# ntu-caokun/DIRECT

Measured on AMD Instinct MI355X. Metric: ddp_iterations_per_sec, higher is better.
Workload: dtype f64

## Files before the change

direct_amd/abi.py:

```python
import ctypes as C

import numpy as np

NX = 9
NU = 10
P_LIMIT = 128

DIRECT_OK = 0
DIRECT_ERR_INVALID = 1
DIRECT_ERR_UNSUPPORTED = 2
DIRECT_ERR_DEVICE = 3
DIRECT_ERR_NO_DEVICE = 4

F32 = 0
F64 = 1
MEM_HOST = 0
MEM_DEVICE = 1

RTN_DONE = 0
RTN_FEAS_OPT = 1
RTN_FEAS_FOUND = 2
RTN_NEG_TIME = -3
RTN_BP_STUCK = -4
RTN_INVALID = -100
# ... 170 lines not shown
class ClusterCorridorOut(C.Structure):
    _fields_ = [("mem", C.c_int32), ("reserved", C.c_int32), ("n_seg", C.c_void_p), ("n_planes", C.c_void_p), ("planes", C.c_void_p),
                ("seeds", C.c_void_p), ("centers", C.c_void_p), ("rtn", C.c_void_p)]


CLUSTER_CORRIDOR_OUTPUTS = ("n_seg", "n_planes", "planes", "seeds", "centers", "rtn")
CLUSTER_CORRIDOR_ARGTYPES = (C.c_void_p, C.c_void_p, C.c_void_p, C.c_void_p)
CLUSTER_CORRIDOR_STATS = ("rounds", "due_seeds", "unique_seeds", "pops")


class LaunchInfo(C.Structure):
    _fields_ = [
        ("dynamic", C.c_int32), ("shared_search", C.c_int32), ("pair_trials", C.c_int32), ("single_steps", C.c_int32),
        ("n_buffers", C.c_int32), ("resident_waves", C.c_int32), ("batch", C.c_int32), ("shared_sweep", C.c_int32),
        ("bwd_knot_visits", C.c_uint64), ("fwd_knot_visits", C.c_uint64),
        ("half_tickets", C.c_int32), ("reserved", C.c_int32),
    ]


class Config(C.Structure):
    _fields_ = [
        ("dtype", C.c_int32), ("device", C.c_int32), ("max_batch", C.c_int32),
        ("n_seg_max", C.c_int32), ("p_max", C.c_int32), ("reserved", C.c_int32),
    ]


FLAG_STATIC_SCHEDULE, FLAG_YIELD = 1, 2


def phase0_params(**kw):
    d = dict(max_vel=2.0, max_acc=2.0, w_snap=1.0, w_terminal=1.0, w_time=1.0, iter_max=50,
# ... 119 lines not shown
```

direct_amd/csrc/ddp_wave.h:

```cpp
#pragma once
#include <stdint.h>

#include "ddp_tables.h"
#include "sched_ticket.h"

#if defined(DIRECT_EMULATE)
#include <cmath>
#include <cstdio>
#include <cstdlib>
#include <cstring>
namespace direct {
using std::fabs; using std::fma; using std::fmax; using std::fmin; using std::log; using std::pow; using std::sqrt;
inline int& emu_lane() { static thread_local int l = 64; return l; }
template <typename T>
inline T* uniform_ptr(T* p) { return p; }
template <typename T>
inline T emu_uniform(T x, int line) {
  static thread_local unsigned char seen[4096][sizeof(double)];
  const int l = emu_lane();
  if (l >= 64) return x;
  unsigned char* ref = seen[line & 4095];
  if (l == 0) {
    std::memcpy(ref, &x, sizeof(T));
  } else if (std::memcmp(ref, &x, sizeof(T)) != 0 && !(x != x)) {
// ... 1075 lines not shown
      if (lane < 9) L.z[lane] = ldx(Xp(buf, N), lane) - (Real)B.xd[(size_t)b * 9 + lane];
    }
    WSYNC();
    const double pterm = terminal_sq();
    WSYNC();
    LANES { LV(slog) = LV(plog).value(); }
    st.costq = qsum;
    st.cost = qsum + 0.5 * B.k.w_term * pterm;
    st.sumlog = WAVE_SUM_D(slog);
    st.errsum = WAVE_SUM_D(serr);
    st.viol = WAVE_SUM_I(nviol);
    st.npos = WAVE_SUM_I(npos);
    st.neg_time = neg;
  }

  DDP_DEV void reset_filter() {
    double logcost = st.cost - st.mu * st.sumlog;
    double err = 0.0;
    if (st.infeas) {
      err = st.errsum;
      if (err < B.k.tol) err = 0.0;
    }
    st.logcost = logcost;
    st.err = err;
    double* f = B.filt + (size_t)b * B.fcap * 2;
    f[0] = logcost;
    f[1] = err;
    st.nfilter = 1;
    st.step = 0;
    st.fp_failed = 0;
// ... 44 lines not shown
          Tk = (Real)2 * Tk;
          cnt++;
        } else {
          vio = 0;
        }
        WSYNC();
      }
      LANES {
        if (lane >= 9 && lane < 18) stx(Xp(0, l), lane, L.z[lane]);
        if (lane == 18) stx(Xp(0, l), 18, Tk);
      }
      WSYNC();
    }
  }

  DDP_DEV void begin() {
    N = B.n_seg[b];
    int bad_sizes = (N < 1 || N > B.nmax) ? 1 : 0;
    if (!bad_sizes) {
      PLV(int, badp);
      LANES {
        LV(badp) = 0;
        for (int k = lane; k < N; k += 64) {
          const int np = np_(k);
          if (np < 1 || np > B.pmax || np > Lds::kPMax) LV(badp) = 1;
        }
      }
      bad_sizes = WAVE_ANY(badp);
    }
    if (bad_sizes) {
      N = 0;
      LANES {
        int* dst = (int*)&L.st;
        for (int e = lane; e < (int)(sizeof(TrajState) / 4); e += 64) dst[e] = 0;
      }
      WSYNC();
      st.rtn = -100;
      st.done = 1;
      st.line_failed = 1;
      return;
    }
    st.nseg = N;
    st.cur = 0;
    st.infeas = B.infeas_in ? (int)B.infeas_in[b] : 0;
    st.infeas_ref = st.infeas;
    st.line_failed = 1;
    const St* T0 = B.T0 + (size_t)b * B.nmax;
    LANES {
      if (lane < 9) stx(Xp(0, 0), lane, (Real)B.x0[(size_t)b * 9 + lane]);
      for (int k = lane; k < N; k += 64) {
        St* rec = Xp(0, k);
        Real T = T0[k];
        if (B.k.zero_init || (B.init_bez == nullptr && B.init_poly == nullptr)) {
          for (int a = 0; a < 9; a++) stx(rec, 9 + a, (Real)0);
        } else if (B.init_poly != nullptr) {
          const St* row = B.init_poly + ((size_t)b * B.nmax + k) * 18;
          for (int a = 0; a < 9; a++) stx(rec, 9 + a, (Real)row[9 + a]);
        } else {
          const St* row = B.init_bez + ((size_t)b * B.nmax + k) * 18;
          for (int i = 3; i < 6; i++)
            for (int d = 0; d < 3; d++) {
              Real acc = 0;
              for (int l = 0; l < 6; l++) acc += (Real)kBez2Mono[l][i] * (T * (Real)row[d * 6 + l]);
              stx(rec, 9 + (i - 3) * 3 + d, acc / powi(T, i));
            }
        }
        stx(rec, 18, T);
      }
    }
    if (!B.k.zero_init && B.k.line_init) line_init();
    for (int k = 0; k < N; k++) {
      const int nc = 6 * np_(k) + 55;
      LANES {
        for (int i = 0; i < RPL; i++) {
          int r = lane + 64 * i;
          if (r < nc) {
            Sp_(B.S[0], k)[r] = (St)0.1;
            Sp_(B.Y[0], k)[r] = (St)0.01;
          }
        }
      }
    }
    WSYNC();
    eval_sweep(0, true);
    if (B.k.line_init && st.npos == 0 && st.infeas) {
      st.infeas = 0;
      eval_sweep(0, false);
    }
    st.prev_cost = st.cost;
    st.nc0 = 6 * np_(0) + 55;
    st.mu = st.cost / (double)N / (double)st.nc0;
    reset_filter();
    st.reg = B.k.line_init ? 10 : 0;
    st.bp_failed = 0;
    st.opterr = 0.0;
    st.stepsize = 0.0;
    st.rtn = 0;
    st.iter = 0;
    st.done = 0;
    st.bp_no_upd = 0;
    st.no_upd = 0;
    st.fwd_passes = 0;
// ... 2463 lines not shown
```

direct_amd/csrc/direct_ddp.hip:

```cpp
#include <hip/hip_runtime.h>

#include <cmath>
#include <cstdio>
#include <cstdlib>
#include <cstring>
#include <string>
#include <vector>

#include "../../include/direct_ddp.h"
#include "ddp_wave.h"
#include "traj_sample.h"
#include "traj_eval.h"
#include "traj_audit.h"
#include "corridor_io.h"
#include "host_stage.h"
#include "rccl_gather.h"

using namespace direct;

#if defined(DDP_TIMING)
#undef DDP_TICK_OBJ
#define DDP_TICK_OBJ W
#endif
#ifndef DDP_WAVES_F32
// ... 7 lines not shown
#define DDP_WAVES_WIDE 2
#endif
#ifndef DDP_WAVES_WIDER
#define DDP_WAVES_WIDER 1
#endif
template <typename St>
struct MinWaves { static constexpr int v = DDP_WAVES_F32; };
template <>
struct MinWaves<double> { static constexpr int v = DDP_WAVES_F64; };

template <typename St>
__device__ __forceinline__ int traj_of(const Batch<St>& B, int i) {
  return B.idx ? __builtin_amdgcn_readfirstlane(B.idx[i]) : i;
}

template <typename St, int RPL>
__global__ __launch_bounds__(64) void k_begin(Batch<St> B) {
  __shared__ WaveLds<Cmp, St, RPL> lds;
  Wave<Cmp, St, RPL> W(B, lds, traj_of(B, blockIdx.x));
  W.init_tables();
  W.begin();
  W.store_state();
}

template <typename St, int RPL>
__global__ __launch_bounds__(64, (RPL > 7 ? DDP_WAVES_WIDER : (RPL > 4 ? DDP_WAVES_WIDE : MinWaves<St>::v))) void k_iterate(Batch<St> B, int n_iters) {
  __shared__ WaveLds<Cmp, St, RPL> lds;
  Wave<Cmp, St, RPL> W(B, lds, traj_of(B, blockIdx.x));
  W.load_state();
  if (__builtin_amdgcn_readfirstlane(lds.st.done)) return;
  W.init_tables();
  W.iterate(n_iters);
  W.store_state();
}

constexpr int kDoneBit = 1 << 30;
#ifndef DDP_POLL_SLEEP
// ... 219 lines not shown
}

template <typename St, int RPL>
__global__ __launch_bounds__(64) void k_stuck(Batch<St> B) {
  __shared__ WaveLds<Cmp, St, RPL> lds;
  Wave<Cmp, St, RPL> W(B, lds, traj_of(B, blockIdx.x));
  W.load_state();
  if (__builtin_amdgcn_readfirstlane(lds.st.rtn) != kRtnStuckPending) return;
  W.init_tables();
  W.stuck_tail();
  W.store_state();
}

template <typename St, int RPL>
__global__ __launch_bounds__(64) void k_finish(Batch<St> B, OutPtrs<St> O, const int* sched_err) {
  __shared__ WaveLds<Cmp, St, RPL> lds;
  Wave<Cmp, St, RPL> W(B, lds, traj_of(B, blockIdx.x));
  W.load_state();
  W.init_tables();
  if (__builtin_amdgcn_readfirstlane(*sched_err)) lds.st.rtn = -101;
  finish_wave(W, O);
}

template <typename St, int RPL>
__global__ __launch_bounds__(64) void k_field(Batch<St> B, int field, St* buf, int set) {
  __shared__ WaveLds<Cmp, St, RPL> lds;
  Wave<Cmp, St, RPL> W(B, lds, traj_of(B, blockIdx.x));
  W.load_state();
  W.init_tables();
  if (set) {
// ... 163 lines not shown
  int* live = nullptr;
  unsigned long long* visits = nullptr;
  direct_ddp_launch_info_t last_info = {};
  int sched_slots = 0;
  int slots_cap = 0;
  int sched_chunk = 1;
  int sched_half = -1;
  int pair_trials = -1;
  int sched_prio = 1;
  int sched_tail = 8;
  int yield_k = 0;
  int* nwaves = nullptr;
  int* sched_dbg = nullptr;
  int* sched_mark = nullptr;
  bool dynamic = true;
  int B = 0;
  bool begun = false;
  direct_ddp_params_t params = {};
  direct_ddp_batch_in_t cur_in = {};
  std::vector<void*> allocs;
};

template <typename T>
static direct_status_t dalloc(direct_ddp_handle_t h, T** p, size_t bytes) {
  hipError_t e = hs::alloc_all(h->allocs, {hs::want(p, bytes)});
  if (e != hipSuccess) return fail(DIRECT_ERR_DEVICE, std::string("hipMalloc: ") + hipGetErrorString(e));
  return DIRECT_OK;
}
#define TRY(expr)                            \
  do {                                       \
// ... 88 lines not shown
  switch (rpl) {
#define OCC_CASE(R) case R: e = hipOccupancyMaxActiveBlocksPerMultiprocessor(&per_cu, k_iterate_dyn<Real, R>, 64, 0); break;
    OCC_CASE(2) OCC_CASE(3) OCC_CASE(4) OCC_CASE(5) OCC_CASE(6) OCC_CASE(7) OCC_CASE(8) OCC_CASE(10) OCC_CASE(12)
#undef OCC_CASE
    default: e = hipOccupancyMaxActiveBlocksPerMultiprocessor(&per_cu, k_iterate_dyn<Real, 14>, 64, 0);
  }
#endif
  int v = (e == hipSuccess && per_cu > 0) ? per_cu * h->n_cu : 0;
  if (h->slots_cap > 0 && v > h->slots_cap) v = h->slots_cap;
  h->slots_of[rpl] = v > 0 ? v : -1;
  return v;
}

template <typename Real>
static void launch_begin_t(direct_ddp_handle_t h) {
  for (const auto& c : batch_classes(h)) {
    auto Bt = make_batch<Real>(h, h->cur_in, h->params, c);
    RPL_LAUNCH(c.rpl, h->stream, k_begin, Real, c.cnt, Bt);
  }
}
static hipStream_t class_stream(direct_ddp_handle_t h, size_t ci, size_t n_classes) {
  if (n_classes <= 1 || ci >= 12) return h->stream;
  if (!h->fork_ev && hipEventCreateWithFlags(&h->fork_ev, hipEventDisableTiming) != hipSuccess) return h->stream;
  if (!h->cstream[ci]) {
    if (hipStreamCreateWithFlags(&h->cstream[ci], hipStreamNonBlocking) != hipSuccess ||
        hipEventCreateWithFlags(&h->cev[ci], hipEventDisableTiming) != hipSuccess) {
      h->cstream[ci] = nullptr;
      return h->stream;
    }
  }
  return h->cstream[ci];
}
template <typename Real>
static void launch_iterate_t(direct_ddp_handle_t h, int n, int mode) {
  const auto classes = batch_classes(h);
  (void)hipMemsetAsync(h->visits, 0, 4 * sizeof(unsigned long long), h->stream);
  direct_ddp_launch_info_t& li = h->last_info;
  li = direct_ddp_launch_info_t{};
  li.n_buffers = h->nbuf; li.batch = h->B;
  if (mode == 0) {
    (void)hipMemsetAsync(h->tickets, 0, 16 * sizeof(int), h->stream);
    (void)hipMemsetAsync(h->sched + 2, 0, (size_t)h->B * sizeof(int), h->stream);
    if (h->help) (void)hipMemsetAsync(h->help, 0, (size_t)h->B * sizeof(HelpSlot), h->stream);
    if (h->bshare && h->bshare_mode != 0) {
      const size_t nb = (size_t)(h->B < h->bshare_cap ? h->B : h->bshare_cap);
      (void)hipMemsetAsync(h->bshare, 0, nb * sizeof(BwdShare), h->stream);
      (void)hipMemsetAsync(h->bflag, 0, nb * h->nmax * sizeof(int), h->stream);
    }
  }
  bool forked = false;
  if (mode == 0 && classes.size() > 1 && class_stream(h, 0, classes.size()) != h->stream) {
    (void)hipEventRecord(h->fork_ev, h->stream);
    forked = true;
  }
  int biggest = -1;
  for (size_t ci = 0; ci < classes.size(); ci++) {
    const auto& c = classes[ci];
    auto Bt = make_batch<Real>(h, h->cur_in, h->params, c);
// ... 55 lines not shown
      S.half = h->sched_half > 0 ? 1 : 0;
      S.chunk = S.half ? 1 : h->sched_chunk;
      S.prio = h->sched_prio;
      S.tail = help ? h->sched_tail : 0;
      S.dbg = h->sched_dbg;
#if defined(DDP_SCHED_DEBUG)
      S.mark = nullptr; S.grid = slots;
      if (slots <= 8192) { S.mark = h->sched_mark; Bt.mark = h->sched_mark; (void)hipMemsetAsync(h->sched_mark, 0, 2 * 8192 * sizeof(int), st); }
#endif
      S.waves = h->nwaves + (ci < 16 ? ci : 15);
      S.alive = h->live + (ci < 16 ? ci : 15);
      S.yield_k = h->yield_k;
      S.yield_min = 64;
      if (h->yield_k > 0) {
        S.tail = 0;
        (void)hipMemsetD32Async((hipDeviceptr_t)S.waves, slots, 1, st);
        (void)hipMemsetD32Async((hipDeviceptr_t)S.alive, c.cnt, 1, st);
      }
      if (help) {
        Bt.help = h->help;
        Bt.help_early = h->help_early;
        int* live = h->live + (ci < 16 ? ci : 15);
        (void)hipMemsetD32Async((hipDeviceptr_t)live, c.cnt, 1, st);
        Bt.live = live;
        Bt.tail_thresh = h->single_ratio > 0 ? slots / h->single_ratio : 0;
        if (is_big) { li.shared_search = 1; li.single_steps = Bt.k.pair_trials ? 0 : 1; }
        if (sweep_ok && h->bshare_mode != 0 && h->bshare_mode != 2 && S.chunk == 1 && (h->bshare_mode > 0 || 8 * c.cnt <= slots)) {
          Bt.bshare = h->bshare; Bt.bflag = h->bflag; Bt.brec = h->brec; Bt.bforce = 0; Bt.bvisits = h->visits + 2;
          if (is_big) li.shared_sweep = 1;
        }
      }
      if (is_big) { li.dynamic = 1; li.half_tickets = S.half; }
      if (Bt.bshare) {
        publish(Bt);
        switch (c.rpl) {
          case 2: hipLaunchKernelGGL((k_iterate_dyn<Real, 2, true>), dim3(slots), dim3(64), 0, st, Bt, n, S); break;
#if !defined(DDP_DEV_RPL2)
          case 3: hipLaunchKernelGGL((k_iterate_dyn<Real, 3, true>), dim3(slots), dim3(64), 0, st, Bt, n, S); break;
          default: hipLaunchKernelGGL((k_iterate_dyn<Real, 4, true>), dim3(slots), dim3(64), 0, st, Bt, n, S);
#endif
        }
      } else {
        RPL_LAUNCH(c.rpl, st, k_iterate_dyn, Real, slots, Bt, n, S);
      }
    } else {
      Bt.bshare = nullptr;
      if (is_big && li.shared_sweep) li.shared_sweep = 0;
      RPL_LAUNCH(c.rpl, st, k_iterate, Real, c.cnt, Bt, n);
    }
    {
      auto Bs = make_batch<Real>(h, h->cur_in, h->params, c);
      Bs.visits = h->visits;
      RPL_LAUNCH(c.rpl, st, k_stuck, Real, c.cnt, Bs);
    }
    if (forked && st != h->stream) {
      (void)hipEventRecord(h->cev[ci], st);
      (void)hipStreamWaitEvent(h->stream, h->cev[ci], 0);
    }
  }
}
template <typename Real>
static void launch_field_t(direct_ddp_handle_t h, int field, int set) {
  for (const auto& c : batch_classes(h)) {
    auto Bt = make_batch<Real>(h, h->cur_in, h->params, c);
    RPL_LAUNCH(c.rpl, h->stream, k_field, Real, c.cnt, Bt, field, (Real*)h->fieldbuf, set);
// ... 5 lines not shown
  const bool dev = out->mem == DIRECT_MEM_DEVICE;
#define PICK(f) (dev ? out->f : (out->f ? h->o.f : nullptr))
  O.rtn = PICK(rtn); O.iter_used = PICK(iter_used); O.fwd_passes = PICK(fwd_passes);
  O.infeas_out = PICK(infeas_out); O.line_failed_out = PICK(line_failed_out);
  O.cost = (Real*)PICK(cost); O.costq = (Real*)PICK(costq); O.jerk_cost = (Real*)PICK(jerk_cost);
  O.terminal_norm2 = (Real*)PICK(terminal_norm2); O.opterr = (Real*)PICK(opterr); O.mu = (Real*)PICK(mu);
  O.bez = (Real*)PICK(bez); O.poly = (Real*)PICK(poly); O.T = (Real*)PICK(T);
#undef PICK
  return O;
}
template <typename Real>
static void launch_finish_t(direct_ddp_handle_t h, const direct_ddp_batch_out_t* out) {
  auto O = out_ptrs<Real>(h, out);
  for (const auto& c : batch_classes(h)) {
    auto Bt = make_batch<Real>(h, h->cur_in, h->params, c);
    RPL_LAUNCH(c.rpl, h->stream, k_finish, Real, c.cnt, Bt, O, (const int*)(h->sched + 1));
  }
}

static direct_status_t staged_upload(direct_ddp_handle_t h, hs::Stage& st, const char* name) {
  const hipError_t e = hs::stage_upload(st, h->stage, h->stream);
  return e == hipSuccess ? DIRECT_OK : fail(DIRECT_ERR_DEVICE, std::string(name) + ": staging: " + hipGetErrorString(e));
}
static direct_status_t staged_finish(direct_ddp_handle_t h, const hs::Stage& st, const char* name) {
  hipError_t e = hs::stage_download(st, h->stream, hipGetLastError());
  if (st.host) e = hs::drain(h->stream, e);
  return e == hipSuccess ? DIRECT_OK : fail(DIRECT_ERR_DEVICE, std::string(name) + ": " + hipGetErrorString(e));
}
static direct_status_t workspace(direct_ddp_handle_t h, hs::Block& ws, size_t bytes, const char* name) {
  const hipError_t e = hs::grow(ws, h->stream, bytes);
  return e == hipSuccess ? DIRECT_OK : fail(DIRECT_ERR_DEVICE, std::string("workspace of ") + name + ": " + hipGetErrorString(e));
// ... 225 lines not shown
  A(&h->best_idx, 16); A(&h->best_cost, 16);
  A(&h->sched, (B + 2) * sizeof(int));
  A(&h->visits, 4 * sizeof(unsigned long long));
  A(&h->live, 16 * sizeof(int));
  A(&h->nwaves, 16 * sizeof(int));
  A(&h->sched_mark, 2 * 8192 * sizeof(int));
  A(&h->sched_dbg, 64 * sizeof(int));
  if (st == DIRECT_OK && hipMemset(h->sched_dbg, 0, 64 * sizeof(int)) != hipSuccess) st = fail(DIRECT_ERR_DEVICE, "hipMemset");
  A(&h->tickets, 16 * sizeof(int));
  A(&h->order, B * sizeof(int32_t)); A(&h->cls_dev, B * sizeof(int32_t));
  if (const char* ev = getenv("DIRECT_DDP_CHUNK")) h->sched_chunk = atoi(ev) > 0 ? atoi(ev) : 1;
  if (const char* ev = getenv("DIRECT_DDP_HALF")) h->sched_half = atoi(ev) > 0 ? 1 : 0;
  if (const char* ev = getenv("DIRECT_DDP_PRIO")) h->sched_prio = atoi(ev);
  if (const char* ev = getenv("DIRECT_DDP_TAIL")) h->sched_tail = std::max(0, std::min(atoi(ev), 64));
  if (const char* ev = getenv("DIRECT_DDP_PAIR")) h->pair_trials = atoi(ev);
  h->fieldbuf_bytes = B * nm * (size_t)std::max(ncm, 100) * r + B * 16 * r + B * 9 * r;
  A(&h->fieldbuf, h->fieldbuf_bytes);
  if (st == DIRECT_OK && (hipEventCreate(&h->ev0) != hipSuccess || hipEventCreate(&h->ev1) != hipSuccess ||
                          hs::create(h->sample_ev) != hipSuccess || hs::create(h->eval_ev) != hipSuccess ||
                          hs::create(h->audit_ev) != hipSuccess))
    st = fail(DIRECT_ERR_DEVICE, "hipEventCreate failed");
  if (st == DIRECT_OK && hipMemset(h->sched, 0, (B + 2) * sizeof(int)) != hipSuccess)
    st = fail(DIRECT_ERR_DEVICE, "hipMemset failed");
  if (st != DIRECT_OK) {
    direct_ddp_destroy(h);
    return st;
  }
  *out = h;
  return DIRECT_OK;
}
// ... 132 lines not shown
    HIP_TRY(up(h->x0, in->x0, B * 9 * r)); d.x0 = h->x0;
    HIP_TRY(up(h->xd, in->xd, B * 9 * r)); d.xd = h->xd;
    if (in->T0) { HIP_TRY(up(h->T0, in->T0, B * nm * r)); d.T0 = h->T0; }
    HIP_TRY(up(h->n_planes, in->n_planes, B * nm * 4)); d.n_planes = h->n_planes;
    HIP_TRY(up(h->planes, in->planes, B * nm * h->pmax * 4 * r)); d.planes = h->planes;
    if (in->init_bez) { HIP_TRY(up(h->init_bez, in->init_bez, B * nm * 18 * r)); d.init_bez = h->init_bez; }
    if (in->init_poly) { HIP_TRY(up(h->init_poly, in->init_poly, B * nm * 18 * r)); d.init_poly = h->init_poly; }
    if (in->seeds) { HIP_TRY(up(h->seeds, in->seeds, B * nm * 3 * r)); d.seeds = h->seeds; }
    if (in->infeas_in) { HIP_TRY(up(h->infeas_in, in->infeas_in, B)); d.infeas_in = h->infeas_in; }
    if (packed) {
      HIP_TRY(hipMemcpyAsync(h->in_blob, h->in_host, h->in_blob_bytes, hipMemcpyHostToDevice, h->stream));
      HIP_TRY(hipEventRecord(h->in_ev, h->stream));
      h->in_ev_pending = true;
    }
  }
  if (!in->infeas_in) {
    HIP_TRY(hipMemsetAsync(h->infeas_in, p->infeas ? 1 : 0, B, h->stream));
    d.infeas_in = h->infeas_in;
  }
  if (!in->T0) {
    const int n = (int)(B * nm);
    if (h->dtype == DIRECT_F64)
      hipLaunchKernelGGL(k_time_alloc<double>, dim3((n + 255) / 256), dim3(256), 0, h->stream, (int)B, (int)nm, d.n_seg, (const double*)d.x0,
                         (const double*)d.xd, (const double*)d.seeds, p->max_vel, p->max_acc, (double*)h->T0);
    else
      hipLaunchKernelGGL(k_time_alloc<float>, dim3((n + 255) / 256), dim3(256), 0, h->stream, (int)B, (int)nm, d.n_seg, (const float*)d.x0,
                         (const float*)d.xd, (const float*)d.seeds, p->max_vel, p->max_acc, (float*)h->T0);
    HIP_TRY(hipGetLastError());
    d.T0 = h->T0;
  }
  if (fresh) {
    h->B = in->batch;
    TRY(classify_batch(h, in->mem == DIRECT_MEM_HOST ? in : &d, in->mem == DIRECT_MEM_HOST));
  }
  if (fresh) HIP_TRY(hipMemsetAsync(h->sched + 1, 0, sizeof(int), h->stream));
  d.mem = DIRECT_MEM_DEVICE;
  h->cur_in = d;
  h->params = *p;
  h->B = in->batch;
  if (p->iter_max + 4 > h->fcap) {
    if (h->filt) { HIP_TRY(hipStreamSynchronize(h->stream)); HIP_TRY(hipFree(h->filt)); h->filt = nullptr; }
    h->fcap = p->iter_max + 4;
    HIP_TRY(hipMalloc((void**)&h->filt, (size_t)h->max_batch * h->fcap * 2 * sizeof(double)));
  }
  return DIRECT_OK;
}

static direct_status_t launch_begin(direct_ddp_handle_t h) {
  if (h->dtype == DIRECT_F64) launch_begin_t<double>(h);
  else launch_begin_t<float>(h);
  HIP_TRY(hipGetLastError());
  h->begun = true;
  return DIRECT_OK;
}

static direct_status_t launch_iterate(direct_ddp_handle_t h, int n, int mode) {
  if (!h->begun) return fail(DIRECT_ERR_INVALID, "direct_ddp_begin has not been called");
  HIP_TRY(hipEventRecord(h->ev0, h->stream));
  if (h->dtype == DIRECT_F64) launch_iterate_t<double>(h, n, mode);
  else launch_iterate_t<float>(h, n, mode);
  HIP_TRY(hipGetLastError());
  HIP_TRY(hipEventRecord(h->ev1, h->stream));
  h->n_launches = 1;
  h->timed = true;
  return DIRECT_OK;
}

static direct_status_t launch_finish(direct_ddp_handle_t h, direct_ddp_batch_out_t* out) {
  if (!h->begun) return fail(DIRECT_ERR_INVALID, "direct_ddp_begin has not been called");
  if (!out) return fail(DIRECT_ERR_INVALID, "null out");
  if (h->dtype == DIRECT_F64) launch_finish_t<double>(h, out);
  else launch_finish_t<float>(h, out);
// ... 53 lines not shown
}
direct_status_t direct_ddp_iterate(direct_ddp_handle_t h, int32_t n_iters) {
  if (!h) return fail(DIRECT_ERR_INVALID, "null handle");
  return launch_iterate(h, n_iters, 0);
}
direct_status_t direct_ddp_finish(direct_ddp_handle_t h, direct_ddp_batch_out_t* out) {
  if (!h) return fail(DIRECT_ERR_INVALID, "null handle");
  return launch_finish(h, out);
}

direct_status_t direct_ddp_solve_batch(direct_ddp_handle_t h, const direct_ddp_params_t* params,
                                       const direct_ddp_batch_in_t* in, direct_ddp_batch_out_t* out) {
  if (!out) return fail(DIRECT_ERR_INVALID, "null out");
  TRY(stage_inputs(h, params, in));
  TRY(launch_begin(h));
  TRY(launch_iterate(h, params->iter_max, 0));
  return launch_finish(h, out);
}

direct_status_t direct_ddp_plan_batch(direct_ddp_handle_t h, const direct_ddp_params_t* p0, const direct_ddp_params_t* p1,
                                      const direct_ddp_batch_in_t* in, direct_ddp_batch_out_t* out0,
                                      direct_ddp_batch_out_t* out1) {
  if (!h || !out1 || !in || !p0 || !p1) return fail(DIRECT_ERR_INVALID, "null argument");
  TRY(check_params(p0));
  TRY(check_params(p1));
  direct_ddp_batch_in_t in0 = *in;
  in0.infeas_in = nullptr;
  direct_ddp_params_t q0 = *p0;
  q0.infeas = 1;
  TRY(stage_inputs(h, &q0, &in0));
  TRY(launch_begin(h));
  TRY(launch_iterate(h, q0.iter_max, 0));
  direct_ddp_batch_out_t stage = {};
  stage.mem = DIRECT_MEM_DEVICE;
  stage.rtn = h->o.rtn; stage.iter_used = h->o.iter_used; stage.fwd_passes = h->o.fwd_passes;
  stage.infeas_out = h->o.infeas_out; stage.line_failed_out = h->o.line_failed_out;
  stage.cost = h->o.cost; stage.costq = h->o.costq; stage.jerk_cost = h->o.jerk_cost;
  stage.terminal_norm2 = h->o.terminal_norm2; stage.opterr = h->o.opterr; stage.mu = h->o.mu;
  stage.bez = h->o.bez; stage.poly = h->o.poly; stage.T = h->o.T;
  TRY(launch_finish(h, &stage));
  const bool out0_packed = out0 && out0->mem == DIRECT_MEM_HOST && h->out_blob != nullptr;
  if (out0_packed) {
    HIP_TRY(hipMemcpyAsync(h->out0_host, h->out_blob, h->out_blob_bytes, hipMemcpyDeviceToHost, h->stream));
  } else if (out0) {
    const size_t B = h->B, nm = h->nmax, r = h->rsz;
    hipMemcpyKind kind = out0->mem == DIRECT_MEM_HOST ? hipMemcpyDeviceToHost : hipMemcpyDeviceToDevice;
    auto cp = [&](void* dst, const void* src, size_t bytes) { return dst ? hipMemcpyAsync(dst, src, bytes, kind, h->stream) : hipSuccess; };
// ... 11 lines not shown
    hipLaunchKernelGGL(k_chain<double>, dim3((n + 255) / 256), dim3(256), 0, h->stream, h->B, h->nmax, h->o.rtn,
                       (const double*)h->o.T, (const double*)h->cur_in.T0, h->o.infeas_out, (const double*)h->o.poly,
                       (double*)h->T_next, h->infeas_next, (double*)h->init_poly);
  else
    hipLaunchKernelGGL(k_chain<float>, dim3((n + 255) / 256), dim3(256), 0, h->stream, h->B, h->nmax, h->o.rtn,
                       (const float*)h->o.T, (const float*)h->cur_in.T0, h->o.infeas_out, (const float*)h->o.poly,
                       (float*)h->T_next, h->infeas_next, (float*)h->init_poly);
  HIP_TRY(hipGetLastError());
  direct_ddp_batch_in_t in1 = h->cur_in;
  in1.T0 = h->T_next;
  in1.init_bez = nullptr;
  in1.init_poly = h->init_poly;
  in1.infeas_in = h->infeas_next;
  TRY(stage_inputs(h, p1, &in1, false));
  TRY(launch_begin(h));
  TRY(launch_iterate(h, p1->iter_max, 0));
  const direct_status_t fin = launch_finish(h, out1);
  if (out0_packed) {
    if (out1->mem != DIRECT_MEM_HOST || fin != DIRECT_OK) HIP_TRY(hipStreamSynchronize(h->stream));
    const size_t B = h->B, nm = h->nmax, r = h->rsz;
    auto sc = [&](void* dst, const void* src, size_t bytes) {
      if (dst) memcpy(dst, h->out0_host + ((const char*)src - h->out_blob), bytes);
    };
    sc(out0->rtn, h->o.rtn, B * 4); sc(out0->iter_used, h->o.iter_used, B * 4); sc(out0->fwd_passes, h->o.fwd_passes, B * 4);
    sc(out0->infeas_out, h->o.infeas_out, B); sc(out0->line_failed_out, h->o.line_failed_out, B);
    sc(out0->cost, h->o.cost, B * r); sc(out0->costq, h->o.costq, B * r); sc(out0->jerk_cost, h->o.jerk_cost, B * r);
    sc(out0->terminal_norm2, h->o.terminal_norm2, B * r); sc(out0->opterr, h->o.opterr, B * r); sc(out0->mu, h->o.mu, B * r);
    sc(out0->bez, h->o.bez, B * nm * 18 * r); sc(out0->poly, h->o.poly, B * nm * 18 * r); sc(out0->T, h->o.T, B * nm * r);
  }
  return fin;
}
// ... 427 lines not shown
```

include/direct_ddp.h:

```cpp
#ifndef DIRECT_DDP_H_
#define DIRECT_DDP_H_

#include <stddef.h>
#include <stdint.h>

#ifdef __cplusplus
extern "C" {
#endif

#define DIRECT_DDP_ABI_VERSION 1

#define DIRECT_NX 9
#define DIRECT_NU 10
#define DIRECT_P_LIMIT 128

typedef enum {
  DIRECT_OK = 0,
  DIRECT_ERR_INVALID = 1,
  DIRECT_ERR_UNSUPPORTED = 2,
  DIRECT_ERR_DEVICE = 3,
  DIRECT_ERR_NO_DEVICE = 4
} direct_status_t;

typedef enum { DIRECT_F32 = 0, DIRECT_F64 = 1 } direct_dtype_t;
// ... 230 lines not shown

direct_status_t direct_ddp_last_kernel_ms(direct_ddp_handle_t h, double* ms, int32_t* n_launches);

typedef struct {
  int32_t dynamic;
  int32_t shared_search;
  int32_t pair_trials;
  int32_t single_steps;
  int32_t n_buffers;
  int32_t resident_waves;
  int32_t batch;
  int32_t shared_sweep;
  uint64_t bwd_knot_visits;
  uint64_t fwd_knot_visits;
  int32_t half_tickets;
  int32_t reserved;
} direct_ddp_launch_info_t;
direct_status_t direct_ddp_last_launch_info(direct_ddp_handle_t h, direct_ddp_launch_info_t* info);
direct_status_t direct_ddp_last_counters(direct_ddp_handle_t h, uint64_t* out4);

direct_status_t direct_ddp_best_cost(direct_ddp_handle_t h, int32_t mem, const void* cost,
                                     const int32_t* rtn, int32_t batch, int32_t* best_index,
                                     double* best_cost);

typedef struct { char internal[128]; } direct_rccl_id_t;
direct_status_t direct_rccl_unique_id(direct_rccl_id_t* id);
direct_status_t direct_rccl_comm_create(direct_ddp_handle_t h, const direct_rccl_id_t* id, int32_t n_ranks,
                                        int32_t rank, void** comm);
direct_status_t direct_rccl_comm_destroy(void* comm);
direct_status_t direct_ddp_gather_best(direct_ddp_handle_t h, void* nccl_comm, int32_t n_ranks, int32_t rank,
                                       int32_t mem, const void* cost, const int32_t* rtn, const void* bez,
// ... 8 lines not shown
```

Baseline: 2.592 million.

## Fuse per-step memsets into begin kernel, fold stuck pass into finish, prefetch eval sweep

Scheduler state resets (tickets, done epochs, help slots, live and wave counters, visit counters, sched error, infeas defaults) move out of separate hipMemset calls and into the begin kernel or a single reset kernel. When finish directly follows iterate, the separate k_stuck launch is skipped and the stuck tail runs inside k_finish. The initial eval sweep gains a software-prefetched variant that loads the next knot's state, planes and duals one step ahead, and per-knot np lookups are batched across lanes. The aim is to cut launch and memset overhead per solve, at the cost of more complex state-reset logic, with a legacy path kept behind an environment variable.

```diff
diff --git a/direct_amd/abi.py b/direct_amd/abi.py
--- a/direct_amd/abi.py
+++ b/direct_amd/abi.py
@@ -208,7 +208,7 @@
         ("dynamic", C.c_int32), ("shared_search", C.c_int32), ("pair_trials", C.c_int32), ("single_steps", C.c_int32),
         ("n_buffers", C.c_int32), ("resident_waves", C.c_int32), ("batch", C.c_int32), ("shared_sweep", C.c_int32),
         ("bwd_knot_visits", C.c_uint64), ("fwd_knot_visits", C.c_uint64),
-        ("half_tickets", C.c_int32), ("reserved", C.c_int32),
+        ("half_tickets", C.c_int32), ("fused_step", C.c_int32),
     ]
 
 
diff --git a/direct_amd/csrc/ddp_wave.h b/direct_amd/csrc/ddp_wave.h
--- a/direct_amd/csrc/ddp_wave.h
+++ b/direct_amd/csrc/ddp_wave.h
@@ -1113,6 +1113,146 @@
     st.neg_time = neg;
   }
 
+  struct EvPre {
+    St zh, zl, pl[kNPL], y[RPL];
+  };
+  template <bool INFEAS>
+  DDP_DEV void ev_prefetch(EvPre& p, int lane, int buf, int k, int P) const {
+    const St* rec = Xp(buf, k);
+    const int a = lane < 19 ? lane : 18;
+    p.zh = rec[a];
+    p.zl = (sizeof(St) < sizeof(double)) ? rec[19 + a] : (St)0;
+    const St* pk = planes_(k);
+    const int pend = 4 * P - 1;
+    for (int i = 0; i < kNPL; i++) p.pl[i] = pk[lane + 64 * i < pend ? lane + 64 * i : pend];
+    if (INFEAS) {
+      const St* yk = Sp_(B.Y[buf], k);
+      for (int i = 0; i < RPL; i++) {
+        if (!slot_on(i, P)) continue;
+        const int r = (row_pack(i, lane, P) & kRMask) - 1;
+        p.y[i] = yk[r >= 0 ? r : 0];
+      }
+    }
+  }
+  template <bool INFEAS>
+  DDP_DEV void ev_pin(EvPre& p) const {
+#if !defined(DIRECT_EMULATE) && !defined(DDP_NO_PREFETCH_PIN)
+    DDP_PIN(p.zh);
+    if (sizeof(St) < sizeof(double)) DDP_PIN(p.zl);
+#pragma unroll
+    for (int i = 0; i < kNPL; i++) DDP_PIN(p.pl[i]);
+    if (INFEAS) {
+#pragma unroll
+      for (int i = 0; i < RPL; i++) DDP_PIN(p.y[i]);
+    }
+#else
+    (void)p;
+#endif
+  }
+  template <bool INFEAS>
+  DDP_DEV void eval_sweep_pre_t(int buf, bool do_roll) {
+    PLV(LogProd<Real>, plog);
+    PLV(Real, slog);
+    PLV(Real, serr);
+    PLV(int, nviol);
+    PLV(int, npos);
+    LANES { LV(plog).init(); LV(serr) = 0; LV(nviol) = 0; LV(npos) = 0; }
+    double qsum = 0.0;
+    int neg = 0;
+    PLV(int, npv);
+    PLV(int, npn);
+    LANES {
+      LV(npv) = np_(lane < N ? lane : N - 1);
+      LV(npn) = np_(64 + lane < N ? 64 + lane : N - 1);
+    }
+    PLV(EvPre, pre);
+    int Pn = RDLANE_I(npv, 0);
+    LANES { ev_prefetch<INFEAS>(LV(pre), lane, buf, 0, Pn); }
+    for (int k = 0; k < N; k++) {
+      const int P = Pn;
+      PLA(Real, yv, RPL);
+      LANES {
+        const bool rolled = do_roll && k > 0 && lane < 9;
+        Real zr = (Real)LV(pre).zh;
+        if (sizeof(St) < sizeof(double)) zr += (Real)LV(pre).zl;
+        if (lane < 19) L.z[lane] = rolled ? pair_round(L.ft[0].xnx[lane]) : zr;
+        for (int i = 0; i < kNPL; i++)
+          if (lane + 64 * i < 4 * P) L.pl[lane + 64 * i] = (Real)LV(pre).pl[i];
+        if (INFEAS) {
+          for (int i = 0; i < RPL; i++) {
+            if (!slot_on(i, P)) continue;
+            LV(yv)[i] = (Real)LV(pre).y[i];
+          }
+        }
+      }
+      {
+        const int kn = k + 1 < N ? k + 1 : N - 1;
+        if ((kn & 63) == 0 && kn != k) {
+          LANES {
+            LV(npv) = LV(npn);
+            LV(npn) = np_(kn + 64 + lane < N ? kn + 64 + lane : N - 1);
+          }
+        }
+        Pn = RDLANE_I(npv, kn & 63);
+        LANES { ev_prefetch<INFEAS>(LV(pre), lane, buf, kn, Pn); }
+      }
+      WSYNC();
+      const Real T = L.z[18];
+      if (T < 0) neg = 1;
+      LANES { if (lane < 8) L.tp[lane] = powi(T, lane); }
+      WSYNC();
+      LANES {
+        if (lane < 45) L.val[lane] = ctrl_val(L.z, L.tp, lane / 3, lane % 3);
+        else if (lane < 54) { if (do_roll) L.ft[0].xnx[lane - 45] = next_x(L.z, L.tp, lane - 45); }
+        else if (lane < 63) L.ft[0].qp[lane - 54] = jerk_part(L.z, L.tp, lane - 54);
+        else L.val[45] = T;
+      }
+      WSYNC();
+      qsum += knot_cost(T, L.ft[0].qp);
+      LANES {
+        for (int i = 0; i < RPL; i++) {
+          if (!slot_on(i, P)) continue;
+          const RowK<Real> rk = row_slot(i, lane, P);
+          const int r = rk.r;
+          if (r >= 0) {
+            Real c = row_c(L.val, rk);
+            if (INFEAS) {
+              Real y = LV(yv)[i];
+              LV(plog).mul(y);
+              LV(serr) += fabs(c + y);
+            } else {
+              LV(plog).mul(-c);
+            }
+            if (c >= (Real)2.0e-4) LV(nviol)++;
+            if (c > (Real)0) LV(npos)++;
+          }
+        }
+        LV(plog).norm();
+        ev_pin<INFEAS>(LV(pre));
+        if (do_roll && lane < 9) stx(Xp(buf, k + 1), lane, L.ft[0].xnx[lane]);
+      }
+      WSYNC();
+    }
+    LANES {
+      if (lane < 9) L.z[lane] = ldx(Xp(buf, N), lane) - (Real)B.xd[(size_t)b * 9 + lane];
+    }
+    WSYNC();
+    const double pterm = terminal_sq();
+    WSYNC();
+    LANES { LV(slog) = LV(plog).value(); }
+    st.costq = qsum;
+    st.cost = qsum + 0.5 * B.k.w_term * pterm;
+    st.sumlog = WAVE_SUM_D(slog);
+    st.errsum = WAVE_SUM_D(serr);
+    st.viol = WAVE_SUM_I(nviol);
+    st.npos = WAVE_SUM_I(npos);
+    st.neg_time = neg;
+  }
+  DDP_DEV void eval_sweep_pre(int buf, bool do_roll) {
+    if (DDP_UNIFORM_I(st.infeas)) eval_sweep_pre_t<true>(buf, do_roll);
+    else eval_sweep_pre_t<false>(buf, do_roll);
+  }
+
   DDP_DEV void reset_filter() {
     double logcost = st.cost - st.mu * st.sumlog;
     double err = 0.0;
@@ -1187,7 +1327,8 @@
     }
   }
 
-  DDP_DEV void begin() {
+  template <bool PRE = true>
+  DDP_DEV void begin(int infeas_default = 0) {
     N = B.n_seg[b];
     int bad_sizes = (N < 1 || N > B.nmax) ? 1 : 0;
     if (!bad_sizes) {
@@ -1215,7 +1356,7 @@
     }
     st.nseg = N;
     st.cur = 0;
-    st.infeas = B.infeas_in ? (int)B.infeas_in[b] : 0;
+    st.infeas = B.infeas_in ? (int)B.infeas_in[b] : infeas_default;
     st.infeas_ref = st.infeas;
     st.line_failed = 1;
     const St* T0 = B.T0 + (size_t)b * B.nmax;
@@ -1228,13 +1369,22 @@
           for (int a = 0; a < 9; a++) stx(rec, 9 + a, (Real)0);
         } else if (B.init_poly != nullptr) {
           const St* row = B.init_poly + ((size_t)b * B.nmax + k) * 18;
-          for (int a = 0; a < 9; a++) stx(rec, 9 + a, (Real)row[9 + a]);
+          if (PRE) {
+            Real uw[9];
+            for (int a = 0; a < 9; a++) uw[a] = (Real)row[9 + a];
+            for (int a = 0; a < 9; a++) stx(rec, 9 + a, uw[a]);
+          } else {
+            for (int a = 0; a < 9; a++) stx(rec, 9 + a, (Real)row[9 + a]);
+          }
         } else {
           const St* row = B.init_bez + ((size_t)b * B.nmax + k) * 18;
+          Real rw[18];
+          if (PRE)
+            for (int l = 0; l < 18; l++) rw[l] = (Real)row[l];
           for (int i = 3; i < 6; i++)
             for (int d = 0; d < 3; d++) {
               Real acc = 0;
-              for (int l = 0; l < 6; l++) acc += (Real)kBez2Mono[l][i] * (T * (Real)row[d * 6 + l]);
+              for (int l = 0; l < 6; l++) acc += (Real)kBez2Mono[l][i] * (T * (PRE ? rw[d * 6 + l] : (Real)row[d * 6 + l]));
               stx(rec, 9 + (i - 3) * 3 + d, acc / powi(T, i));
             }
         }
@@ -1242,23 +1392,45 @@
       }
     }
     if (!B.k.zero_init && B.k.line_init) line_init();
-    for (int k = 0; k < N; k++) {
-      const int nc = 6 * np_(k) + 55;
-      LANES {
-        for (int i = 0; i < RPL; i++) {
-          int r = lane + 64 * i;
-          if (r < nc) {
-            Sp_(B.S[0], k)[r] = (St)0.1;
-            Sp_(B.Y[0], k)[r] = (St)0.01;
+    if (PRE) {
+      for (int k0 = 0; k0 < N; k0 += 64) {
+        PLV(int, npc);
+        LANES { LV(npc) = np_(k0 + lane < N ? k0 + lane : N - 1); }
+        const int kc = N - k0 < 64 ? N - k0 : 64;
+        for (int j = 0; j < kc; j++) {
+          const int nc = 6 * RDLANE_I(npc, j) + 55;
+          LANES {
+            for (int i = 0; i < RPL; i++) {
+              int r = lane + 64 * i;
+              if (r < nc) {
+                Sp_(B.S[0], k0 + j)[r] = (St)0.1;
+                Sp_(B.Y[0], k0 + j)[r] = (St)0.01;
+              }
+            }
+          }
+        }
+      }
+    } else {
+      for (int k = 0; k < N; k++) {
+        const int nc = 6 * np_(k) + 55;
+        LANES {
+          for (int i = 0; i < RPL; i++) {
+            int r = lane + 64 * i;
+            if (r < nc) {
+              Sp_(B.S[0], k)[r] = (St)0.1;
+              Sp_(B.Y[0], k)[r] = (St)0.01;
+            }
           }
         }
       }
     }
     WSYNC();
-    eval_sweep(0, true);
+    if (PRE) eval_sweep_pre(0, true);
+    else eval_sweep(0, true);
     if (B.k.line_init && st.npos == 0 && st.infeas) {
       st.infeas = 0;
-      eval_sweep(0, false);
+      if (PRE) eval_sweep_pre_t<false>(0, false);
+      else eval_sweep(0, false);
     }
     st.prev_cost = st.cost;
     st.nc0 = 6 * np_(0) + 55;
diff --git a/direct_amd/csrc/direct_ddp.hip b/direct_amd/csrc/direct_ddp.hip
--- a/direct_amd/csrc/direct_ddp.hip
+++ b/direct_amd/csrc/direct_ddp.hip
@@ -45,13 +45,71 @@
   return B.idx ? __builtin_amdgcn_readfirstlane(B.idx[i]) : i;
 }
 
+struct StepReset {
+  int* done_epoch;
+  HelpSlot* help;
+  unsigned long long* visits;
+  int* tickets;
+  int* sched_err;
+  int* live;
+  int* waves;
+  int live_n, waves_n;
+  int infeas_default;
+};
+constexpr int kHelpWords = (int)(sizeof(HelpSlot) / sizeof(int));
+static_assert(sizeof(HelpSlot) % sizeof(int) == 0, "HelpSlot is cleared word by word");
+__device__ __forceinline__ void reset_scalars(const StepReset& R, int lane) {
+  if (R.visits != nullptr && lane < 4) R.visits[lane] = 0ull;
+  if (R.tickets != nullptr && lane < 16) R.tickets[lane] = 0;
+  if (lane == 0) {
+    if (R.sched_err != nullptr) *R.sched_err = 0;
+    if (R.live != nullptr) *R.live = R.live_n;
+    if (R.waves != nullptr) *R.waves = R.waves_n;
+  }
+}
+
 template <typename St, int RPL>
-__global__ __launch_bounds__(64) void k_begin(Batch<St> B) {
+__global__ __launch_bounds__(64) void k_begin(Batch<St> B, StepReset R) {
+  __shared__ WaveLds<Cmp, St, RPL> lds;
+  const int b = traj_of(B, blockIdx.x);
+  Wave<Cmp, St, RPL> W(B, lds, b);
+  if (R.done_epoch != nullptr && threadIdx.x == 0) R.done_epoch[b] = 0;
+  if (R.help != nullptr) {
+    int* hs = (int*)&R.help[b];
+    for (int e = threadIdx.x; e < kHelpWords; e += 64) hs[e] = 0;
+  }
+  if (blockIdx.x == 0) reset_scalars(R, threadIdx.x);
+  W.init_tables();
+  W.begin(R.infeas_default);
+  W.store_state();
+}
+template <typename St, int RPL>
+__global__ __launch_bounds__(64) void k_begin_legacy(Batch<St> B) {
   __shared__ WaveLds<Cmp, St, RPL> lds;
   Wave<Cmp, St, RPL> W(B, lds, traj_of(B, blockIdx.x));
   W.init_tables();
-  W.begin();
+  W.template begin<false>();
   W.store_state();
+}
+struct ResetClasses {
+  int n;
+  int live_n[16], waves_n[16];
+};
+__global__ __launch_bounds__(256) void k_reset(StepReset R, int batch, int all, ResetClasses C) {
+  const int i = blockIdx.x * blockDim.x + threadIdx.x, stride = gridDim.x * blockDim.x;
+  if (i < 4 && R.visits != nullptr) R.visits[i] = 0ull;
+  if (!all) return;
+  if (i < 16 && R.tickets != nullptr) R.tickets[i] = 0;
+  if (i < C.n) {
+    if (R.live != nullptr) R.live[i] = C.live_n[i];
+    if (R.waves != nullptr) R.waves[i] = C.waves_n[i];
+  }
+  if (R.done_epoch != nullptr)
+    for (int e = i; e < batch; e += stride) R.done_epoch[e] = 0;
+  if (R.help != nullptr) {
+    int* hs = (int*)R.help;
+    for (long long e = i; e < (long long)batch * kHelpWords; e += stride) hs[e] = 0;
+  }
 }
 
 template <typename St, int RPL>
@@ -301,6 +359,20 @@
 
 template <typename St, int RPL>
 __global__ __launch_bounds__(64) void k_finish(Batch<St> B, OutPtrs<St> O, const int* sched_err) {
+  __shared__ WaveLds<Cmp, St, RPL> lds;
+  Wave<Cmp, St, RPL> W(B, lds, traj_of(B, blockIdx.x));
+  W.load_state();
+  W.init_tables();
+  if (__builtin_amdgcn_readfirstlane(lds.st.rtn) == kRtnStuckPending) {
+    W.stuck_tail();
+    W.store_state();
+    WSYNC();
+  }
+  if (__builtin_amdgcn_readfirstlane(*sched_err)) lds.st.rtn = -101;
+  finish_wave(W, O);
+}
+template <typename St, int RPL>
+__global__ __launch_bounds__(64) void k_finish_legacy(Batch<St> B, OutPtrs<St> O, const int* sched_err) {
   __shared__ WaveLds<Cmp, St, RPL> lds;
   Wave<Cmp, St, RPL> W(B, lds, traj_of(B, blockIdx.x));
   W.load_state();
@@ -494,6 +566,11 @@
   int* sched_dbg = nullptr;
   int* sched_mark = nullptr;
   bool dynamic = true;
+  bool legacy_step = false;
+  bool step_clean = false;
+  bool err_fresh = false;
+  int infeas_default = 0;
+  bool finish_follows = false;
   int B = 0;
   bool begun = false;
   direct_ddp_params_t params = {};
@@ -612,10 +689,52 @@
 
 template <typename Real>
 static void launch_begin_t(direct_ddp_handle_t h) {
-  for (const auto& c : batch_classes(h)) {
+  const auto classes = batch_classes(h);
+  for (size_t ci = 0; ci < classes.size(); ci++) {
+    const auto& c = classes[ci];
     auto Bt = make_batch<Real>(h, h->cur_in, h->params, c);
-    RPL_LAUNCH(c.rpl, h->stream, k_begin, Real, c.cnt, Bt);
-  }
+    if (h->legacy_step) {
+      RPL_LAUNCH(c.rpl, h->stream, k_begin_legacy, Real, c.cnt, Bt);
+      continue;
+    }
+    StepReset R = {};
+    R.done_epoch = h->sched + 2;
+    R.help = h->help;
+    if (ci == 0) {
+      R.visits = h->visits;
+      R.tickets = h->tickets;
+      R.sched_err = h->err_fresh ? h->sched + 1 : nullptr;
+    }
+    const size_t cs = ci < 16 ? ci : 15;
+    R.live = h->live + cs; R.live_n = c.cnt;
+    if (h->yield_k > 0) { R.waves = h->nwaves + cs; R.waves_n = resident_slots<Real>(h, c.rpl); }
+    R.infeas_default = h->infeas_default;
+    RPL_LAUNCH(c.rpl, h->stream, k_begin, Real, c.cnt, Bt, R);
+  }
+  h->step_clean = !h->legacy_step;
+}
+template <typename Real>
+static void launch_reset_t(direct_ddp_handle_t h, int all) {
+  const auto classes = batch_classes(h);
+  StepReset R = {};
+  ResetClasses C = {};
+  R.visits = h->visits;
+  if (all) {
+    R.done_epoch = h->sched + 2;
+    R.help = h->help;
+    R.tickets = h->tickets;
+    R.live = h->live;
+    if (h->yield_k > 0) R.waves = h->nwaves;
+    C.n = (int)(classes.size() < 16 ? classes.size() : 16);
+    for (size_t ci = 0; ci < classes.size(); ci++) {
+      const size_t cs = ci < 16 ? ci : 15;
+      C.live_n[cs] = classes[ci].cnt;
+      C.waves_n[cs] = resident_slots<Real>(h, classes[ci].rpl);
+    }
+  }
+  const long long words = all ? (long long)h->B * (h->help ? kHelpWords : 1) : 4;
+  const int grid = (int)std::min<long long>((words + 255) / 256, 1024);
+  hipLaunchKernelGGL(k_reset, dim3(grid), dim3(256), 0, h->stream, R, h->B, all, C);
 }
 static hipStream_t class_stream(direct_ddp_handle_t h, size_t ci, size_t n_classes) {
   if (n_classes <= 1 || ci >= 12) return h->stream;
@@ -632,14 +751,21 @@
 template <typename Real>
 static void launch_iterate_t(direct_ddp_handle_t h, int n, int mode) {
   const auto classes = batch_classes(h);
-  (void)hipMemsetAsync(h->visits, 0, 4 * sizeof(unsigned long long), h->stream);
+  const bool fused = !h->legacy_step;
+  const bool clean = fused && h->step_clean;
+  h->step_clean = false;
+  if (!fused) (void)hipMemsetAsync(h->visits, 0, 4 * sizeof(unsigned long long), h->stream);
+  else if (!clean) launch_reset_t<Real>(h, mode == 0 ? 1 : 0);
   direct_ddp_launch_info_t& li = h->last_info;
   li = direct_ddp_launch_info_t{};
   li.n_buffers = h->nbuf; li.batch = h->B;
+  li.fused_step = fused ? 1 : 0;
   if (mode == 0) {
-    (void)hipMemsetAsync(h->tickets, 0, 16 * sizeof(int), h->stream);
-    (void)hipMemsetAsync(h->sched + 2, 0, (size_t)h->B * sizeof(int), h->stream);
-    if (h->help) (void)hipMemsetAsync(h->help, 0, (size_t)h->B * sizeof(HelpSlot), h->stream);
+    if (!fused) {
+      (void)hipMemsetAsync(h->tickets, 0, 16 * sizeof(int), h->stream);
+      (void)hipMemsetAsync(h->sched + 2, 0, (size_t)h->B * sizeof(int), h->stream);
+      if (h->help) (void)hipMemsetAsync(h->help, 0, (size_t)h->B * sizeof(HelpSlot), h->stream);
+    }
     if (h->bshare && h->bshare_mode != 0) {
       const size_t nb = (size_t)(h->B < h->bshare_cap ? h->B : h->bshare_cap);
       (void)hipMemsetAsync(h->bshare, 0, nb * sizeof(BwdShare), h->stream);
@@ -725,14 +851,16 @@
       S.yield_min = 64;
       if (h->yield_k > 0) {
         S.tail = 0;
-        (void)hipMemsetD32Async((hipDeviceptr_t)S.waves, slots, 1, st);
-        (void)hipMemsetD32Async((hipDeviceptr_t)S.alive, c.cnt, 1, st);
+        if (!fused) {
+          (void)hipMemsetD32Async((hipDeviceptr_t)S.waves, slots, 1, st);
+          (void)hipMemsetD32Async((hipDeviceptr_t)S.alive, c.cnt, 1, st);
+        }
       }
       if (help) {
         Bt.help = h->help;
         Bt.help_early = h->help_early;
         int* live = h->live + (ci < 16 ? ci : 15);
-        (void)hipMemsetD32Async((hipDeviceptr_t)live, c.cnt, 1, st);
+        if (!fused) (void)hipMemsetD32Async((hipDeviceptr_t)live, c.cnt, 1, st);
         Bt.live = live;
         Bt.tail_thresh = h->single_ratio > 0 ? slots / h->single_ratio : 0;
         if (is_big) { li.shared_search = 1; li.single_steps = Bt.k.pair_trials ? 0 : 1; }
@@ -759,7 +887,7 @@
       if (is_big && li.shared_sweep) li.shared_sweep = 0;
       RPL_LAUNCH(c.rpl, st, k_iterate, Real, c.cnt, Bt, n);
     }
-    {
+    if (!(fused && h->finish_follows)) {
       auto Bs = make_batch<Real>(h, h->cur_in, h->params, c);
       Bs.visits = h->visits;
       RPL_LAUNCH(c.rpl, st, k_stuck, Real, c.cnt, Bs);
@@ -795,7 +923,12 @@
   auto O = out_ptrs<Real>(h, out);
   for (const auto& c : batch_classes(h)) {
     auto Bt = make_batch<Real>(h, h->cur_in, h->params, c);
-    RPL_LAUNCH(c.rpl, h->stream, k_finish, Real, c.cnt, Bt, O, (const int*)(h->sched + 1));
+    if (h->legacy_step) {
+      RPL_LAUNCH(c.rpl, h->stream, k_finish_legacy, Real, c.cnt, Bt, O, (const int*)(h->sched + 1));
+    } else {
+      Bt.visits = h->visits;
+      RPL_LAUNCH(c.rpl, h->stream, k_finish, Real, c.cnt, Bt, O, (const int*)(h->sched + 1));
+    }
   }
 }
 
@@ -1051,6 +1184,7 @@
   if (const char* ev = getenv("DIRECT_DDP_PRIO")) h->sched_prio = atoi(ev);
   if (const char* ev = getenv("DIRECT_DDP_TAIL")) h->sched_tail = std::max(0, std::min(atoi(ev), 64));
   if (const char* ev = getenv("DIRECT_DDP_PAIR")) h->pair_trials = atoi(ev);
+  if (const char* ev = getenv("DIRECT_DDP_LEGACY_STEP")) h->legacy_step = atoi(ev) != 0;
   h->fieldbuf_bytes = B * nm * (size_t)std::max(ncm, 100) * r + B * 16 * r + B * 9 * r;
   A(&h->fieldbuf, h->fieldbuf_bytes);
   if (st == DIRECT_OK && (hipEventCreate(&h->ev0) != hipSuccess || hipEventCreate(&h->ev1) != hipSuccess ||
@@ -1213,7 +1347,8 @@
       h->in_ev_pending = true;
     }
   }
-  if (!in->infeas_in) {
+  h->infeas_default = p->infeas ? 1 : 0;
+  if (!in->infeas_in && h->legacy_step) {
     HIP_TRY(hipMemsetAsync(h->infeas_in, p->infeas ? 1 : 0, B, h->stream));
     d.infeas_in = h->infeas_in;
   }
@@ -1232,7 +1367,8 @@
     h->B = in->batch;
     TRY(classify_batch(h, in->mem == DIRECT_MEM_HOST ? in : &d, in->mem == DIRECT_MEM_HOST));
   }
-  if (fresh) HIP_TRY(hipMemsetAsync(h->sched + 1, 0, sizeof(int), h->stream));
+  if (fresh && h->legacy_step) HIP_TRY(hipMemsetAsync(h->sched + 1, 0, sizeof(int), h->stream));
+  h->err_fresh = fresh;
   d.mem = DIRECT_MEM_DEVICE;
   h->cur_in = d;
   h->params = *p;
@@ -1253,8 +1389,9 @@
   return DIRECT_OK;
 }
 
-static direct_status_t launch_iterate(direct_ddp_handle_t h, int n, int mode) {
+static direct_status_t launch_iterate(direct_ddp_handle_t h, int n, int mode, bool finish_follows = false) {
   if (!h->begun) return fail(DIRECT_ERR_INVALID, "direct_ddp_begin has not been called");
+  h->finish_follows = finish_follows;
   HIP_TRY(hipEventRecord(h->ev0, h->stream));
   if (h->dtype == DIRECT_F64) launch_iterate_t<double>(h, n, mode);
   else launch_iterate_t<float>(h, n, mode);
@@ -1338,7 +1475,7 @@
   if (!out) return fail(DIRECT_ERR_INVALID, "null out");
   TRY(stage_inputs(h, params, in));
   TRY(launch_begin(h));
-  TRY(launch_iterate(h, params->iter_max, 0));
+  TRY(launch_iterate(h, params->iter_max, 0, true));
   return launch_finish(h, out);
 }
 
@@ -1354,7 +1491,7 @@
   q0.infeas = 1;
   TRY(stage_inputs(h, &q0, &in0));
   TRY(launch_begin(h));
-  TRY(launch_iterate(h, q0.iter_max, 0));
+  TRY(launch_iterate(h, q0.iter_max, 0, true));
   direct_ddp_batch_out_t stage = {};
   stage.mem = DIRECT_MEM_DEVICE;
   stage.rtn = h->o.rtn; stage.iter_used = h->o.iter_used; stage.fwd_passes = h->o.fwd_passes;
@@ -1396,7 +1533,7 @@
   in1.infeas_in = h->infeas_next;
   TRY(stage_inputs(h, p1, &in1, false));
   TRY(launch_begin(h));
-  TRY(launch_iterate(h, p1->iter_max, 0));
+  TRY(launch_iterate(h, p1->iter_max, 0, true));
   const direct_status_t fin = launch_finish(h, out1);
   if (out0_packed) {
     if (out1->mem != DIRECT_MEM_HOST || fin != DIRECT_OK) HIP_TRY(hipStreamSynchronize(h->stream));
diff --git a/include/direct_ddp.h b/include/direct_ddp.h
--- a/include/direct_ddp.h
+++ b/include/direct_ddp.h
@@ -268,7 +268,7 @@
   uint64_t bwd_knot_visits;
   uint64_t fwd_knot_visits;
   int32_t half_tickets;
-  int32_t reserved;
+  int32_t fused_step;
 } direct_ddp_launch_info_t;
 direct_status_t direct_ddp_last_launch_info(direct_ddp_handle_t h, direct_ddp_launch_info_t* info);
 direct_status_t direct_ddp_last_counters(direct_ddp_handle_t h, uint64_t* out4);
```

Result: no change. 2.607 million, median of 6 (+0.6%).
